# manyeyes/K2TransducerAsr

Hardware: AMD Instinct MI355X
Metric: RTFx (audio-sec/wall-sec) offline Zipformer greedy (higher is better)
Workload: dtype f32

## Files before the change

k2transducerasr_amd/csrc/engine.cpp:

```cpp
#include <cstring>
#include <thread>

#include "engine.h"

#include <climits>
#include <cmath>

namespace k2hip {

namespace {
constexpr int kTailFrames = 19;
}

Engine::Engine(const std::string& weights, const char* overrides, int device) : device_(device) {
    tunables_init_from_env();
    model_.reset(new Model(weights, overrides));
    int n = 0;
    if (hipGetDeviceCount(&n) != hipSuccess || n <= 0)
        failf(K2HIP_ERR_NO_DEVICE, "no HIP device visible: libk2hip has no CPU fallback");
    if (device < 0 || device >= n) failf(K2HIP_ERR_NO_DEVICE, "device %d out of range (have %d)", device, n);
    K2_HIP(hipSetDevice(device));
    model_->upload(device);
    K2_HIP(hipStreamCreateWithFlags(&stream_, hipStreamNonBlocking));
    K2_HIP(hipStreamCreateWithFlags(&stream2_, hipStreamNonBlocking));
// ... 172 lines not shown
    w.dec_table = d_dec_table_;
    return w;
}

void Engine::decoder_table_check(int n_samples, unsigned seed, long long* rows, long long* mismatched) {
    const DecJoinW w = decjoin();
    *rows = 0;
    *mismatched = 0;
    if (!w.dec_table) return;
    const long long V = w.V, n_ctx = (V + 1) * V;
    *rows = n_ctx;
    std::vector<long long> y;
    auto add = [&](long long y0, long long y1) { y.push_back(y0); y.push_back(y1); };
    add(-1, K2HIP_BLANK_ID);
    add(K2HIP_BLANK_ID, K2HIP_BLANK_ID);
    add(-1, V - 1);
    add(V - 1, V - 1);
    unsigned long long st = seed * 6364136223846793005ull + 1442695040888963407ull;
    for (int i = 0; i < n_samples; i++) {
        st = st * 6364136223846793005ull + 1442695040888963407ull;
        const long long cx = (long long)((st >> 20) % (unsigned long long)n_ctx);
        add(cx / V - 1, cx % V);
    }
    const int N = (int)(y.size() / 2);
    long long* d_y = nullptr;
    float* d_out = nullptr;
    K2_HIP(hipMalloc(&d_y, sizeof(long long) * y.size()));
    K2_HIP(hipMalloc(&d_out, sizeof(float) * (size_t)N * w.J));
    std::vector<float> got((size_t)N * w.J), want(w.J);
    try {
        K2_HIP(hipMemcpyAsync(d_y, y.data(), sizeof(long long) * y.size(), hipMemcpyHostToDevice, stream_));
        Ctx t;
        t.stream = stream_;
        decoder_rows_wide(t, w, d_y, N, d_out);
        K2_HIP(hipMemcpyAsync(got.data(), d_out, sizeof(float) * got.size(), hipMemcpyDeviceToHost, stream_));
        K2_HIP(hipStreamSynchronize(stream_));
        for (int n = 0; n < N; n++) {
            const long long row = (y[2 * n] + 1) * V + y[2 * n + 1];
            K2_HIP(copy_blocking(want.data(), w.dec_table + row * w.J, sizeof(float) * w.J, hipMemcpyDeviceToHost));
            for (int k = 0; k < w.J; k++) *mismatched += memcmp(&want[k], &got[(size_t)n * w.J + k], sizeof(float)) != 0;
        }
    } catch (...) {
        (void)hipFree(d_y);
        (void)hipFree(d_out);
        throw;
    }
    (void)hipFree(d_y);
    (void)hipFree(d_out);
}

float* Engine::encoder_embed(const Ctx& c, const float* x, int B, int T, int* T50) {
    const Model& m = *model_;
    const int F0 = 80, T1 = T - 2, T2 = (T1 - 3) / 2 + 1, F2 = (F0 - 3) / 2 + 1, T3 = T2 - 2, F3 = (F2 - 3) / 2 + 1;
    K2_REQUIRE(T3 > 0, "encoder: %d input frames are too few (need >= 9)", T);
    Arena& ar = *c.arena;
    const int D0 = m.cfg().dim[0];
    float* out = ar.take<float>((int64_t)B * T3 * D0);
    int64_t mark = ar.mark();
    float* a1 = ar.take<float>((int64_t)B * T1 * F0 * 8);
    conv0_swoosh(c, x, m.w("encoder_embed.conv.0.weight"), m.w("encoder_embed.conv.0.bias"), a1, B, T, F0);
    c.add_flops(0, 2.0 * B * T1 * (double)F0 * 8 * 9, 0);
    float* a2 = ar.take<float>((int64_t)B * T2 * F2 * 32);
    {
        GemmArgs g;
        g.A = a1; g.W = m.w("encoder_embed.conv.4.weight#ohwi"); g.ldw = 72; g.bias = m.w("encoder_embed.conv.4.bias");
        g.C = a2; g.ldc = 32; g.M = B * T2 * F2; g.N = 32; g.K = 72; g.act = ACT_SWOOSH_R;
        g.cv_Fout = F2; g.cv_Tout = T2; g.cv_Tin = T1; g.cv_Fin = F0; g.cv_C = 8; g.cv_st = 2; g.cv_sf = 2;
        g.seg_len = 24; g.seg_stride = F0 * 8;
        gemm(c, g);
    }
    float* a3 = ar.take<float>((int64_t)B * T3 * F3 * 128);
    {
        GemmArgs g;
        g.A = a2; g.W = m.w("encoder_embed.conv.7.weight#ohwi"); g.ldw = 288; g.bias = m.w("encoder_embed.conv.7.bias");
        g.C = a3; g.ldc = 128; g.M = B * T3 * F3; g.N = 128; g.K = 288; g.act = ACT_SWOOSH_R;
        g.cv_Fout = F3; g.cv_Tout = T3; g.cv_Tin = T2; g.cv_Fin = F2; g.cv_C = 32; g.cv_st = 1; g.cv_sf = 2;
        g.seg_len = 96; g.seg_stride = F2 * 32;
        gemm(c, g);
    }
    const int npix = B * T3 * F3;
    float* dw = ar.take<float>((int64_t)npix * 128);
    dwconv7x7(c, a3, m.w("encoder_embed.convnext.depthwise_conv.weight#kc"), m.w("encoder_embed.convnext.depthwise_conv.bias"),
              dw, B, T3, T3, 3, F3, 128);
    float* hid = ar.take<float>((int64_t)npix * 384);
    linear(c, dw, 128, m.w("encoder_embed.convnext.pointwise_conv1.weight"), m.w("encoder_embed.convnext.pointwise_conv1.bias"),
           hid, 384, npix, 128, 384, ACT_SWOOSH_L);
    linear(c, hid, 384, m.w("encoder_embed.convnext.pointwise_conv2.weight"), m.w("encoder_embed.convnext.pointwise_conv2.bias"),
           a3, 128, npix, 384, 128, ACT_NONE, a3, 128);
    float* lin = ar.take<float>((int64_t)B * T3 * D0);
    linear(c, a3, F3 * 128, m.w("encoder_embed.out.weight#fc"), m.w("encoder_embed.out.bias"), lin, D0, B * T3, F3 * 128, D0);
    biasnorm(c, lin, m.w("encoder_embed.out_norm.bias"), m.w("encoder_embed.out_norm.log_scale"), out, B * T3, D0);
    ar.rewind(mark);
    *T50 = T3;
    return out;
}

const float* Engine::pos_proj_cached(const Ctx& c, int layer, const float* pe, int pe_dim, const float* W, int rows, int ncols) {
    if (c.dry) return nullptr;
    std::lock_guard<std::mutex> lk(cache_mu_);
    const auto key = std::make_pair(layer, rows);
    auto it = pp_cache_.find(key);
    if (it != pp_cache_.end()) return it->second;
    const size_t bytes = sizeof(float) * (size_t)rows * ncols;
    if (pp_cache_bytes_ + bytes > ((size_t)1 << 30)) {
        synchronize();
        for (auto& kv : pp_cache_) (void)hipFree(kv.second);
        pp_cache_.clear();
        pp_cache_bytes_ = 0;
    }
    float* pp = nullptr;
    K2_HIP(hipMalloc(&pp, bytes));
    Ctx plain = c;
    plain.instrument = false;
    plain.gemm_log = nullptr;
    linear(plain, pe, pe_dim, W, nullptr, pp, ncols, rows, pe_dim, ncols);
    K2_HIP(hipStreamSynchronize(c.stream));
    pp_cache_[key] = pp;
    pp_cache_bytes_ += bytes;
    return pp;
}

void Engine::encoder_layer(const Ctx& c, int si, int li, float* x, const float* pe, int B, int T, const LayerTail* tail) {
    const Model& m = *model_;
    const Config& cf = m.cfg();
    const int D = cf.dim[si], F = cf.ff[si], H = cf.heads[si], vh = cf.vhd[si], K = cf.kern[si];
    const int M = B * T, Tp = (T + 3) & ~3, inproj = (2 * cf.qhd[si] + cf.phd[si]) * H, Hc = 3 * D / 4, HV = H * vh;
    char p[96];
    snprintf(p, sizeof p, "encoder.encoders.%d.layers.%d.", si, li);
    auto w = [&](const char* suffix) { return m.w(std::string(p) + suffix); };
    Arena& ar = *c.arena;
    int64_t mark = ar.mark();

    const int F1 = F * 3 / 4, ldcat = F1 + inproj;
    float* cat = ar.take<float>((int64_t)M * ldcat);
    {
        GemmArgs g;
        g.A = x; g.lda = D; g.W = w("#ff1_attn_in.weight"); g.ldw = D; g.bias = w("#ff1_attn_in.bias");
        g.C = cat; g.ldc = ldcat; g.M = M; g.N = ldcat; g.K = D; g.act = ACT_SWOOSH_L; g.act_cols = F1;
        gemm(c, g);
    }
    const float* qkp = cat + F1;
    int gl = li;
    for (int i = 0; i < si; i++) gl += cf.nlayer[i];
    const float* pp = pos_proj_cached(c, gl, pe, cf.pos_dim, w("self_attn_weights.linear_pos.weight"), 2 * T - 1, cf.phd[si] * H);
    float* aw = ar.take<float>((int64_t)H * B * T * Tp);
    attn_scores_softmax(c, qkp, ldcat, pp, aw, B, T, Tp, H);

    float* src = ar.take<float>((int64_t)M * D);
    float* hid = ar.take<float>((int64_t)M * std::max({F * 5 / 4, 3 * Hc, 2 * D}));
    float* tmp = ar.take<float>((int64_t)M * std::max(D, Hc));
    float* tmp2 = ar.take<float>((int64_t)M * std::max(D, Hc));

    auto feed_forward = [&](int k, int Fk, const float* in, float* out) {
        char a[48], b[48], cc[48], d[48];
        snprintf(a, sizeof a, "feed_forward%d.in_proj.weight", k);
        snprintf(b, sizeof b, "feed_forward%d.in_proj.bias", k);
        snprintf(cc, sizeof cc, "feed_forward%d.out_proj.weight", k);
        snprintf(d, sizeof d, "feed_forward%d.out_proj.bias", k);
        linear(c, in, D, w(a), w(b), hid, Fk, M, D, Fk, ACT_SWOOSH_L);
        linear(c, hid, Fk, w(cc), w(d), out, D, M, Fk, D, ACT_NONE, in, D);
    };
    auto self_attn = [&](int k) {
        char a[48], b[48], cc[48], d[48];
        snprintf(a, sizeof a, "self_attn%d.in_proj.weight", k);
        snprintf(b, sizeof b, "self_attn%d.in_proj.bias", k);
        snprintf(cc, sizeof cc, "self_attn%d.out_proj.weight", k);
        snprintf(d, sizeof d, "self_attn%d.out_proj.bias", k);
        linear(c, src, D, w(a), w(b), hid, HV, M, D, HV);
        if (attn_av_out(c, aw, hid, w(cc), w(d), src, B, T, T, Tp, H, vh, D)) return;
        GemmArgs g;
        g.A = aw; g.lda = Tp; g.sA0 = (long long)T * Tp; g.sA1 = (long long)B * T * Tp;
// ... 1276 lines not shown
            g.glu = I(); g.glu_cols = I();
            g.ldm = I(); g.sM0 = L(); g.sM1 = L();
            g.ld_orig = I();
            const int cfg = I(), res_is_C = I();
            const long long oA = L(), oW = L(), oR = L(), oC = L(), oM = L(), oO = L();
            float *A = P(), *W = P(), *bias = P(), *res = P(), *C = P();
            const int* skip = reinterpret_cast<const int*>(P());
            float *mul = P(), *orig = P(), *scale = P();
            int* plan_out = reinterpret_cast<int*>(P());
            K2_REQUIRE(A && W && C && plan_out && buf_bytes[n_bufs - 1] >= 20, "debug_op_run gemm: A, W, C and a plan buffer of 5 ints are needed");
            K2_REQUIRE(!(res_is_C && res), "debug_op_run gemm: res_is_C takes no res buffer");
            K2_REQUIRE(oA >= 0 && oW >= 0 && oR >= 0 && oC >= 0 && oM >= 0 && oO >= 0, "debug_op_run gemm: negative offset");
            if (res_is_C) res = C;
            g.A = A + oA; g.W = W + oW; g.bias = bias; g.res = res ? res + oR : nullptr; g.C = C + oC;
            g.skip_if_zero = skip;
            g.mul = mul ? mul + oM : nullptr;
            g.byp_orig = orig ? orig + oO : nullptr; g.byp_scale = scale;
            GemmForceGuard force(cfg);
            const GemmPlan pl = plan_gemm(g, gemm_force());
            const int rep[5] = {(int)pl.family, pl.idx, pl.BM, pl.BN, pl.mode};
            K2_HIP(copy_blocking(plan_out, rep, sizeof rep, hipMemcpyHostToDevice));
            gemm(c, g);
        } else if (name == "gemm_glu_causal_conv") {
            float *x = P(), *wg = P(), *bg = P(), *pool = P();
            const long long ss = L(), off = L();
            const int* slots = reinterpret_cast<const int*>(P());
            float *wc = P(), *bc = P(), *ww = P(), *bw = P(), *sc = P(), *y = P();
            const int B = I(), Tc = I(), D = I(), K = I();
            int* entry_out = reinterpret_cast<int*>(P());
            K2_REQUIRE(entry_out && buf_bytes[n_bufs - 1] >= 4, "debug_op_run gemm_glu_causal_conv: an entry buffer of 1 int is needed");
            const int entry = glu_conv_ring_entry(B, Tc, D, K);
            K2_HIP(copy_blocking(entry_out, &entry, sizeof entry, hipMemcpyHostToDevice));
            took = gemm_glu_causal_conv(c, x, wg, bg, pool, ss, off, slots, wc, bc, ww, bw, sc, y, B, Tc, D, K);
        } else if (name == "biasnorm") {
            float *x = P(), *bias = P(), *ls = P(), *y = P();
            const int M = I(), D = I();
            biasnorm(c, x, bias, ls, y, M, D);
        } else if (name == "bypass") {
            float *orig = P(), *x = P(), *scale = P(), *y = P();
            const int M = I(), D = I();
            bypass(c, orig, x, scale, y, M, D);
        } else if (name == "biasnorm_bypass") {
            float *x = P(), *orig = P(), *nb = P(), *ls = P(), *scale = P(), *y = P();
            const int M = I(), D = I();
            biasnorm_bypass(c, x, orig, nb, ls, scale, y, M, D);
        } else if (name == "biasnorm_bypass_downsample") {
            float *x = P(), *orig = P(), *nb = P(), *ls = P(), *scale = P(), *y = P(), *bias2 = P(), *xd2 = P();
            const int B = I(), T = I(), D = I(), ds2 = I(), D2 = I();
            biasnorm_bypass_downsample(c, x, orig, nb, ls, scale, y, bias2, xd2, B, T, D, ds2, D2);
        } else if (name == "downsample") {
            float *x = P(), *bias = P(), *y = P();
            const int B = I(), T = I(), D = I(), ds = I(), Din = I();
            downsample(c, x, bias, y, B, T, D, ds, Din);
        } else if (name == "downsample_full") {
            FullDimSegs s;
            s.n = I();
            K2_REQUIRE(s.n >= 1 && s.n <= 8, "debug_op_run downsample_full: %d segments", s.n);
            for (int k = 0; k < s.n; k++) s.ld[k] = I();
            for (int k = 0; k < s.n; k++) s.col1[k] = I();
            s.lz_Td = I(); s.lz_ds = I(); s.lz_Do = I();
            for (int k = 0; k < s.n; k++) s.src[k] = P();
            s.lz_orig = P(); s.lz_xd = P(); s.lz_scale = P();
            float *bias = P(), *y = P();
            const int B = I(), T = I(), D = I(), ds = I();
            downsample_full(c, s, bias, y, B, T, D, ds);
        } else if (name == "upsample_combine") {
            float *orig = P(), *xd = P(), *scale = P(), *y = P();
            const int B = I(), T = I(), Td = I(), D = I(), ds = I(), Dorig = I();
            upsample_combine(c, orig, xd, scale, y, B, T, Td, D, ds, Dorig);
        } else if (name == "upsample_combine_downsample") {
            float *orig = P(), *xd = P(), *scale = P(), *y = P(), *bias2 = P(), *xd2 = P();
            const int B = I(), T = I(), Td = I(), D = I(), ds = I(), Dorig = I(), D2 = I(), ds2 = I();
            upsample_combine_downsample(c, orig, xd, scale, y, bias2, xd2, B, T, Td, D, ds, Dorig, D2, ds2);
        } else if (name == "glu_dwconv1d_swoosh" || name == "glu_dwconv1d_dswish" || name == "dwconv1d_swoosh") {
            float *x = P(), *w = P(), *b = P(), *y = P();
            const int B = I(), T = I(), D = I(), K = I();
            if (name == "glu_dwconv1d_swoosh") glu_dwconv1d_swoosh(c, x, w, b, y, B, T, D, K);
            else if (name == "glu_dwconv1d_dswish") glu_dwconv1d_dswish(c, x, w, b, y, B, T, D, K);
            else dwconv1d_swoosh(c, x, w, b, y, B, T, D, K);
        } else if (name == "dwconv7x7") {
            float *x = P(), *w = P(), *b = P(), *y = P();
            const int B = I(), Tin = I(), Tout = I(), tpad = I(), F = I(), C = I();
            dwconv7x7(c, x, w, b, y, B, Tin, Tout, tpad, F, C);
        } else if (name == "conformer_qprep") {
            float *qkv = P(), *bu = P(), *bv = P(), *qu = P(), *qv = P();
            const int M = I(), D = I();
            const float scaling = F();
            const int ldq = I();
            conformer_qprep(c, qkv, bu, bv, qu, qv, M, D, scaling, ldq);
        } else if (name == "conformer_scores_softmax") {
            float *qu = P(), *qv = P(), *kmat = P();
            const int ldk = I();
            float *pp = P(), *aw = P();
            const int B = I(), H = I(), T = I(), Tp = I(), D = I(), ldq = I();
            float *bu = P(), *bv = P();
            const float scaling = F();
            took = conformer_scores_softmax(c, qu, qv, kmat, ldk, pp, aw, B, H, T, Tp, D, ldq, bu, bv, scaling);
        } else if (name == "conformer_softmax_shift") {
            float *ac = P(), *bd = P();
            const int Z = I(), T = I(), Tp = I(), NPp = I();
            conformer_softmax_shift(c, ac, bd, Z, T, Tp, NPp);
        } else if (name == "conformer_softmax_shift_stream") {
            float *ac = P(), *bd = P();
            const long long* plen = reinterpret_cast<const long long*>(P());
            const int B = I(), H = I(), Tc = I(), left = I(), KLp = I(), NPp = I();
            conformer_softmax_shift_stream(c, ac, bd, plen, B, H, Tc, left, KLp, NPp);
        } else if (name == "slice_rows") {
            float *in = P(), *out = P();
            const int B = I(), Tin = I(), row0 = I(), Tout = I(), D = I();
            slice_rows(c, in, out, B, Tin, row0, Tout, D);
        } else if (name == "dwconv_valid_dswish") {
            float *cat = P(), *w = P(), *bias = P(), *y = P();
            const int B = I(), Tc = I(), D = I(), K = I();
            dwconv_valid_dswish(c, cat, w, bias, y, B, Tc, D, K);
        } else if (name == "z1_pool") {
            float *x = P(), *pool = P();
            const long long ss = L(), avg_off = L(), len_off = L();
            const int* slots = reinterpret_cast<const int*>(P());
            float* out = P();
            const int B = I(), Tc = I(), D = I();
            z1_pool(c, x, pool, ss, avg_off, len_off, slots, out, B, Tc, D);
        } else if (name == "z1_attn") {
            float* qkvp = P();
            const int ld = I();
            float *kcat = P(), *pp = P(), *aw = P();
            const int B = I(), Tc = I(), Lc = I(), KLp = I(), H = I(), A = I();
            z1_attn(c, qkvp, ld, kcat, pp, aw, B, Tc, Lc, KLp, H, A);
        } else if (name == "z1_glu_conv") {
            float *x2 = P(), *pool = P();
            const long long ss = L(), off = L();
            const int* slots = reinterpret_cast<const int*>(P());
            float *w = P(), *bias = P(), *y = P();
            const int B = I(), Tc = I(), D = I(), K = I();
            z1_glu_conv(c, x2, pool, ss, off, slots, w, bias, y, B, Tc, D, K);
        } else if (name == "z1_norm_bypass") {
            float *x = P(), *orig = P(), *le = P(), *bs = P(), *y = P();
            const int M = I(), D = I();
            z1_norm_bypass(c, x, orig, le, bs, y, M, D);
        } else if (name == "z1_attn_downsample") {
            float *x = P(), *query = P(), *y = P();
            const int B = I(), T = I(), Din = I(), ldy = I(), ds = I();
            z1_attn_downsample(c, x, query, y, B, T, Din, ldy, ds);
        } else if (name == "z1_mean") {
            float *x = P(), *mean = P();
            const int B = I(), T = I(), D = I();
            z1_mean(c, x, mean, B, T, D);
        } else if (name == "z1_add_bcast") {
            float *x = P(), *v = P();
            const int B = I(), T = I(), D = I();
            z1_add_bcast(c, x, v, B, T, D);
        } else if (name == "z1_group_rows") {
            float *x = P(), *grp = P();
            const int B = I(), T = I(), Din = I(), ds = I();
            z1_group_rows(c, x, grp, B, T, Din, ds);
        } else if (name == "z1_combine") {
            float* s1 = P();
            const int d1 = I();
            float* s2 = P();
            const int d2 = I();
            float *w1 = P(), *ub = P();
            const int ds = I(), B = I(), T = I(), Td = I();
            float* y = P();
            z1_combine(c, s1, d1, s2, d2, w1, ub, ds, B, T, Td, y);
        } else if (name == "lstm_cell") {
            float* gx = P();
            const long long ldgx = L();
// ... 157 lines not shown
```

k2transducerasr_amd/csrc/gemm.hip:

```cpp
#include <algorithm>
#include <cmath>
#include <cstdlib>
#include <map>
#include <mutex>
#include <type_traits>

#include "kernels.h"

#pragma clang diagnostic ignored "-Winline-asm"

namespace k2hip {

typedef float f32x16 __attribute__((ext_vector_type(16)));
typedef float f32x4 __attribute__((ext_vector_type(4)));

namespace {


__device__ __forceinline__ float fast_softplus(float z) {
    return z > 15.f ? z : __logf(1.0f + __expf(z));
}
__device__ __forceinline__ float apply_act(float v, int act) {
    switch (act) {
        case ACT_SWOOSH_L: return fast_softplus(v - 4.0f) - 0.08f * v - 0.035f;
// ... 1467 lines not shown
    if (ctx.dry) return;
    if (ctx.instrument) K2_HIP(hipEventRecord(ctx.next_event(), ctx.stream));
    const GemmPlan p = plan_gemm(a, gemm_force());
    GemmArgs b = a;
    b.ablate = p.ablate;
    b.xcd_panels = tunables().xcd_panels;
    switch (p.family) {
        case GemmFamily::REG:
            if (p.mode == MODE_CONV) launch_reg<MODE_CONV>(ctx, b, p.idx);
            else if (p.mode == MODE_WKN) launch_reg<MODE_WKN>(ctx, b, p.idx);
            else launch_reg<MODE_PLAIN>(ctx, b, p.idx);
            break;
        case GemmFamily::DMA:
            switch (p.idx) {
#define X(i, bm, bn, wm, wn, nst) case i: launch_dma<bm, bn, wm, wn, nst>(ctx, b); break;
                K2_DMA_TABLE(X)
#undef X
            }
            break;
        case GemmFamily::PIPE:
            switch (p.idx) {
#define X(i, bm, bn, wm, wn, nst) case i: launch_pipe<bm, bn, wm, wn, nst>(ctx, b); break;
                K2_PIPE_TABLE(X)
#undef X
            }
            break;
        case GemmFamily::P16:
            switch (p.idx) {
#define X(i, bm, bn, wm, wn, nst) case i: launch_p16<bm, bn, wm, wn, nst>(ctx, b); break;
                K2_P16_TABLE(X)
#undef X
            }
            break;
        case GemmFamily::RING:
            switch (p.idx) {
#define X(i, bm, bn, ks, nst, lw, pf) case i: launch_ring<bm, bn, ks, nst, lw, pf>(ctx, b); break;
                K2_RING_TABLE(X)
#undef X
            }
            break;
        case GemmFamily::SKINNY3:
            hipLaunchKernelGGL(gemm_f32_mfma_skinny<3>, dim3(cdiv(a.M, 16), 1), dim3(256), 0, ctx.stream, b);
            break;
        case GemmFamily::SKINNY6:
            hipLaunchKernelGGL(gemm_f32_mfma_skinny<6>, dim3(cdiv(a.M, 16), cdiv(a.N, 96)), dim3(256), 0, ctx.stream, b);
            break;
        case GemmFamily::SKINNY6_8:
            hipLaunchKernelGGL((gemm_f32_mfma_skinny<6, 8>), dim3(cdiv(a.M, 16), cdiv(a.N, 96)), dim3(512), 0, ctx.stream, b);
            break;
    }
    K2_HIP(hipGetLastError());
    if (ctx.instrument && ctx.gemm_log)
        ctx.gemm_log->push_back({a.M, a.N, a.K, a.nb0 * a.nb1, a.act, a.res != nullptr, gemm_kind(a, p), 0.f});
    if (ctx.instrument) K2_HIP(hipEventRecord(ctx.next_event(), ctx.stream));
}

bool gemm_glu_causal_conv(const Ctx& ctx, const float* x, const float* wg, const float* bg, float* pool, long long slot_stride, long long off,
                          const int* slots, const float* wc, const float* bc, const float* ww, const float* bw, const float* sc, float* y, int B,
                          int Tc, int D, int K) {
    const int M = B * Tc, N = 2 * D;
    const int entry = glu_conv_ring_entry(B, Tc, D, K);
    if (entry < 0) return false;
    const double fl = 2.0 * M * (double)N * D;
    ctx.add_flops(fl, 2.0 * M * (double)D * (K + (K + 1) / 2), 1);
    if (ctx.dry) return true;
    GemmArgs g;
    g.A = x; g.lda = D; g.W = wg; g.ldw = D; g.bias = bg; g.C = y; g.ldc = D; g.M = M; g.N = N; g.K = D;
    g.cf_pool = pool; g.cf_stride = slot_stride; g.cf_off = off; g.cf_slots = slots;
    g.cf_wc = wc; g.cf_bc = bc; g.cf_ww = ww; g.cf_bw = bw; g.cf_sc = sc; g.cf_Tc = Tc; g.cf_K = K;
    g.xcd_panels = tunables().xcd_panels;
    if (ctx.instrument) K2_HIP(hipEventRecord(ctx.next_event(), ctx.stream));
    if (ctx.instrument && ctx.gemm_log) ctx.gemm_log->push_back({M, N, D, 1, 0, 0, 64, 0.f});
    switch (entry) {
        case 16: launch_ring_conv_entry<16>(ctx, g); break;
        case 17: launch_ring_conv_entry<17>(ctx, g); break;
        case 12: launch_ring_conv_entry<12>(ctx, g); break;
        default: launch_ring_conv_entry<8>(ctx, g); break;
    }
    K2_HIP(hipGetLastError());
    if (ctx.instrument) K2_HIP(hipEventRecord(ctx.next_event(), ctx.stream));
    return true;
}

void linear(const Ctx& ctx, const float* A, int lda, const float* W, const float* bias, float* C, int ldc, int M, int K,
            int N, int act, const float* res, int ldr) {
    GemmArgs g;
    g.A = A; g.lda = lda; g.W = W; g.ldw = K; g.bias = bias; g.C = C; g.ldc = ldc;
    g.M = M; g.N = N; g.K = K; g.act = act; g.res = res; g.ldr = ldr;
    gemm(ctx, g);
}

}
```

k2transducerasr_amd/csrc/kernels.h:

```cpp
#pragma once
#include "common.h"

namespace k2hip {

#ifdef K2HIP_DEV
#define K2HIP_DEV_SWITCH(name, def) int name = def
#else
#define K2HIP_DEV_SWITCH(name, def) static constexpr int name = def
#endif
struct Tunables {
    int no_glu_epilogue = 0;
    int attn_long = 0;
    int no_fused_av = 0;
    int fused_vproj_min_t = 4;
    int no_fused_vproj = 0;
    int no_fused_conv = 0;
    int conformer_gemm_scores = 0;
    int dw7_tiled = 0;
    int dw1d_tt = 0;
    int lstm_seq = 0;
    int greedy_one_part = 0;
    int greedy_parts = 0;
    int beam_launches = 0;
    int beam_parts = 0;
// ... 100 lines not shown

#define K2_PIPE_TABLE(X)                                                                                                       \
    X(0, 128, 64, 64, 32, 3) X(1, 128, 64, 32, 32, 3) X(2, 128, 128, 64, 64, 3) X(3, 128, 128, 64, 32, 3) X(4, 128, 64, 64, 32, 4)  \
    X(5, 64, 64, 32, 32, 3) X(6, 128, 128, 64, 64, 4) X(7, 64, 128, 32, 64, 3) X(8, 128, 128, 32, 32, 3) X(9, 128, 64, 32, 32, 4) \
    X(10, 64, 64, 64, 32, 3) X(11, 64, 64, 32, 64, 3) X(12, 256, 64, 64, 32, 3) X(13, 128, 32, 32, 32, 3) X(14, 128, 32, 64, 32, 3)
#define K2_P16_TABLE(X) X(0, 64, 96, 32, 48, 3) X(1, 128, 96, 64, 48, 3) X(2, 64, 192, 32, 96, 3) X(3, 32, 96, 16, 48, 3)
#define K2_RING_TABLE(X)                                                                                        \
    X(0, 128, 64, 1, 2, 0, 0) X(1, 128, 64, 1, 3, 0, 0) X(2, 128, 64, 1, 2, 0, 1) X(3, 128, 64, 1, 3, 0, 1) X(4, 128, 64, 1, 4, 0, 1)   \
    X(5, 64, 64, 1, 3, 0, 0) X(6, 64, 64, 1, 3, 0, 1) X(7, 64, 64, 1, 4, 0, 1) X(8, 64, 64, 2, 3, 0, 0) X(9, 64, 64, 2, 3, 0, 1)      \
    X(10, 64, 64, 4, 2, 0, 0) X(11, 64, 64, 4, 2, 0, 1) X(12, 32, 64, 2, 3, 0, 0) X(13, 32, 64, 4, 3, 0, 0) X(14, 32, 64, 4, 3, 0, 1)  \
    X(15, 32, 32, 4, 3, 0, 0) X(16, 32, 32, 4, 4, 0, 1) X(17, 64, 32, 4, 3, 0, 0) X(18, 128, 128, 1, 2, 0, 0) X(19, 128, 128, 1, 2, 0, 1) \
    X(20, 64, 128, 1, 3, 0, 0) X(21, 64, 128, 1, 3, 0, 1) X(22, 64, 96, 1, 3, 0, 0) X(23, 64, 96, 1, 3, 0, 1) X(24, 128, 96, 1, 2, 0, 1) \
    X(25, 128, 64, 1, 3, 2, 0) X(26, 128, 64, 1, 3, 2, 1) X(27, 128, 64, 2, 2, 0, 1) X(28, 64, 96, 2, 3, 0, 0) X(29, 64, 96, 2, 2, 0, 0) \
    X(30, 64, 96, 2, 2, 0, 1) X(31, 128, 96, 1, 3, 0, 0) X(32, 128, 96, 1, 3, 0, 1)
struct RingCfg { int BM, BN, KS, NST, LW, PF; };
#define X(i, bm, bn, ks, nst, lw, pf) {bm, bn, ks, nst, lw, pf},
constexpr RingCfg kRing[] = {K2_RING_TABLE(X)};
#undef X
#define K2_DMA_TABLE(X)                                                                                                          \
    X(0, 128, 128, 64, 32, 3) X(5, 128, 64, 32, 32, 2) X(8, 128, 64, 32, 32, 4) X(9, 64, 64, 32, 32, 2) X(10, 64, 64, 32, 32, 3) \
    X(11, 64, 96, 32, 32, 2) X(20, 32, 32, 32, 32, 4) X(21, 32, 64, 32, 32, 4)
#define K2_REG_TABLE(X)                                                                                                           \
    X(0, 128, 128, 64, 32, 32) X(1, 128, 128, 64, 32, 64) X(2, 64, 64, 32, 32, 32) X(3, 64, 64, 32, 32, 64) X(4, 128, 64, 32, 32, 64) \
    X(5, 128, 64, 32, 32, 32) X(12, 128, 32, 32, 32, 32)
enum GemmMode { MODE_PLAIN = 0, MODE_CONV = 1, MODE_WKN = 2 };

enum class GemmFamily { REG, DMA, PIPE, P16, RING, SKINNY3, SKINNY6, SKINNY6_8 };
struct GemmPlan {
    GemmFamily family = GemmFamily::REG;
    int idx = 0;
    int mode = MODE_PLAIN;
    int ablate = 0;
    int BM = 0, BN = 0, waves = 0;
};
struct GemmForce {
    enum Kind { AUTO, CFG, RING, PIPE, P16 } kind = AUTO;
    int idx = -1;
    int ablate = 0;
    bool dma = true;
};
GemmForce decode_gemm_force(int code);
GemmPlan plan_gemm(const GemmArgs& a, const GemmForce& f);
int gemm_kind(const GemmArgs& a, const GemmPlan& p);
int glu_conv_ring_entry(int B, int Tc, int D, int K);
void debug_force_gemm_cfg(int code);
GemmForce gemm_force();
struct GemmForceGuard {
    explicit GemmForceGuard(int code) { debug_force_gemm_cfg(code); }
    ~GemmForceGuard() { debug_force_gemm_cfg(-1); }
    GemmForceGuard(const GemmForceGuard&) = delete;
    GemmForceGuard& operator=(const GemmForceGuard&) = delete;
};
void linear(const Ctx& ctx, const float* A, int lda, const float* W, const float* bias, float* C, int ldc, int M, int K,
            int N, int act = ACT_NONE, const float* res = nullptr, int ldr = 0);

struct RingRef {
    float* pool = nullptr;
    long long slot_stride = 0;
    long long off = 0;
    const int* slots = nullptr;
    const int* chunks = nullptr;
};

void attn_scores_softmax(const Ctx& ctx, const float* qkp, int ld, const float* pp, float* aw, int B, int T, int Tp, int H, int qh = 32,
                         int koff0 = -1, int poff0 = -1);

bool attn_av_out(const Ctx& ctx, const float* aw, const float* v, const float* wout, const float* bias, float* x, int B, int T, int KL, int Tp,
                 int H, int vh, int D);
bool attn_av_out_ring(const Ctx& ctx, const float* aw, const RingRef& vals, const float* newrows, const float* wout, const float* bias, float* x,
                      int B, int T, int KL, int Tp, int H, int vh, int D);
void attn_proj_av_out_ring(const Ctx& ctx, const float* aw, const RingRef& vals, const float* xin, const float* win, const float* bin,
                           const float* wout, const float* bias, float* xout, int B, int T, int KL, int Tp, int H, int vh, int D);

void nonlin_av_out_ring(const Ctx& ctx, const float* aw, const RingRef& cache, const float* hid, int ldh, const float* wout, const float* bias,
                        float* x, int B, int T, int KL, int Tp, int Hc, int D);

void pad_logfloor(const Ctx& ctx, const float* packed, const long long* d_off, const long long* d_len, float* out, int B,
                  long long L);
void pad_logfloor_dense(const Ctx& ctx, const float* feats, long long n_each, float* out, int B, long long L);
void conv0_swoosh(const Ctx& ctx, const float* x, const float* w, const float* b, float* y, int B, int T, int F);
void conv0_pad1_dswish(const Ctx& ctx, const float* x, const float* w, const float* b, float* y, int B, int T, int F);
void dwconv7x7(const Ctx& ctx, const float* x, const float* w_kc, const float* b, float* y, int B, int Tin, int Tout, int tpad,
               int F, int C);
void biasnorm(const Ctx& ctx, const float* x, const float* bias, const float* log_scale, float* y, int M, int D);
void biasnorm_bypass(const Ctx& ctx, const float* x, const float* orig, const float* nbias, const float* log_scale,
                     const float* scale, float* y, int M, int D);
void biasnorm_bypass_downsample(const Ctx& ctx, const float* x, const float* orig, const float* nbias, const float* log_scale, const float* scale,
                                float* y, const float* bias2, float* xd2, int B, int T, int D, int ds2, int D2);
struct LayerTail {
    const float* bias2 = nullptr;
    float* xd2 = nullptr;
    int ds2 = 1, D2 = 0;
};
void bypass(const Ctx& ctx, const float* orig, const float* x, const float* scale, float* y, int M, int D);
void glu_sigmoid(const Ctx& ctx, const float* x, float* y, int M, int D);
void tanh_gate(const Ctx& ctx, const float* x, float* y, int M, int Hc);
void mul_cols(const Ctx& ctx, float* a, const float* x, int ldx, int col0, int M, int N);
void dwconv1d_swoosh(const Ctx& ctx, const float* x, const float* w_kd, const float* b, float* y, int B, int T, int D, int K);
void glu_dwconv1d_swoosh(const Ctx& ctx, const float* x2, const float* w_kd, const float* b, float* y, int B, int T, int D,
                          int K);
void glu_dwconv1d_dswish(const Ctx& ctx, const float* x2, const float* w_kd, const float* b, float* y, int B, int T, int D,
                          int K);
void conv0_nopad_dswish(const Ctx& ctx, const float* x, const float* w, const float* b, float* y, int B, int T, int F);
void lstm_cell(const Ctx& ctx, const float* gx, long long ldgx, const float* gh, int ldgh, float* c, float* hf, int B, int Hh);
void add_inplace(const Ctx& ctx, float* a, const float* b, long long n);
void lstm_cell_rows(const Ctx& ctx, const float* gates, float* c, float* hf, int rows, int Hh);
void lstm_add_frame(const Ctx& ctx, const float* Y, long long SY, const float* hp, long long pstride, int S, float* h, float* x1, int n, int B,
                    int T, int D, int lo, int s);
void lstm_norm_frame(const Ctx& ctx, const float* x1, const float* fp, long long pstride, int S, const float* b2_0, const float* eps0,
                     long long lstride, float* Y, long long SY, int n, int B, int T, int D, int lo, int s);
void gather_rows(const Ctx& ctx, const float* pool, long long slot_stride, long long off, const int* slots, float* out, int B, int width);
void scatter_rows(const Ctx& ctx, float* pool, long long slot_stride, long long off, const int* slots, const float* in, int ldin, int B, int width);
void basicnorm(const Ctx& ctx, const float* x, const float* log_eps, float* y, int M, int D);
void conformer_qprep(const Ctx& ctx, const float* qkv, const float* bias_u, const float* bias_v, float* qu, float* qv, int M,
                     int D, float scaling, int ldq = 0 );
void conformer_softmax_shift_stream(const Ctx& ctx, float* ac, const float* bd, const long long* plen, int B, int H, int Tc, int left,
                                    int KLp, int NPp);
void slice_rows(const Ctx& ctx, const float* in, float* out, int B, int Tin, int row0, int Tout, int D);
void dwconv_valid_dswish(const Ctx& ctx, const float* cat, const float* w_kd, const float* bias, float* y, int B, int Tc, int D, int K);
void conformer_softmax_shift(const Ctx& ctx, float* ac, const float* bd, int Z, int T, int Tp, int NPp);
bool conformer_scores_softmax(const Ctx& ctx, const float* qu, const float* qv, const float* kmat, int ldk, const float* pp, float* aw, int B, int H,
                              int T, int Tp, int D, int ldq = 0, const float* bias_u = nullptr, const float* bias_v = nullptr, float scaling = 1.0f);
void downsample(const Ctx& ctx, const float* x, const float* bias, float* y, int B, int T, int D, int ds, int Din = 0);
void upsample_combine(const Ctx& ctx, const float* orig, const float* xd, const float* scale, float* y, int B, int T,
                      int Td, int D, int ds, int Dorig = 0);
void upsample_combine_downsample(const Ctx& ctx, const float* orig, const float* xd, const float* scale, float* y, const float* bias2,
                                 float* xd2, int B, int T, int Td, int D, int ds, int Dorig, int D2, int ds2);
void convert_channels(const Ctx& ctx, const float* x, float* y, int M, int Din, int Dout);
struct FullDimSegs {
    const float* src[8];
    int ld[8], col1[8], n = 0;
    const float* lz_orig = nullptr;
    const float* lz_xd = nullptr;
    const float* lz_scale = nullptr;
    int lz_Td = 0, lz_ds = 1, lz_Do = 0;
};
void downsample_full(const Ctx& ctx, const FullDimSegs& segs, const float* bias, float* y, int B, int T, int D, int ds);
void copy_cols(const Ctx& ctx, const float* x, int ldx, int xcol0, float* y, int ldy, int ycol0, int M, int n);

struct FbankArgs {
    const float* samples;
    long long n_samples;
    long long utt_stride;
    int n_utts;
    long long n_frames;
    float* feats;
    const float* window;
    const float* melw;
    int frame_len, frame_shift;
    float preemph, input_scale;
    int remove_dc;
    const float* melrange = nullptr;
};
void fbank(const Ctx& ctx, const FbankArgs& a);
void gather_samples(const Ctx& ctx, const float* const* src, const long long* n, float* dst, int B, long long nmax);

struct DecJoinW {
    const float* emb;
    const float* conv;
    int cpg;
    const float* ptab = nullptr;
    const float* dproj_kn;
    const float* dproj_b;
    const float* out_kn;
    const float* out_b;
    const float* dec_table = nullptr;
// ... 205 lines not shown
```

Measured before the change: 23610.

## Fuse ConvNeXt pointwise MLP pair into one persistent MFMA kernel

Replaces the two linear calls of the encoder_embed ConvNeXt block (128->384 with SwooshL, then 384->128 plus residual) with a single persistent kernel. The kernel keeps the 384-wide hidden activations in registers chunk by chunk and streams weight chunks into LDS via double-buffered global_load_lds DMA. It uses fp32 MFMA 32x32x2 and adds the residual in the epilogue. This removes the write and re-read of the npix x 384 hidden buffer and one launch, at the cost of a hand-tuned kernel with inline asm and a fixed channel shape.

Result: no change. 23540 (-0.3%).

```diff
diff --git a/k2transducerasr_amd/csrc/engine.cpp b/k2transducerasr_amd/csrc/engine.cpp
--- a/k2transducerasr_amd/csrc/engine.cpp
+++ b/k2transducerasr_amd/csrc/engine.cpp
@@ -278,11 +278,8 @@
     float* dw = ar.take<float>((int64_t)npix * 128);
     dwconv7x7(c, a3, m.w("encoder_embed.convnext.depthwise_conv.weight#kc"), m.w("encoder_embed.convnext.depthwise_conv.bias"),
               dw, B, T3, T3, 3, F3, 128);
-    float* hid = ar.take<float>((int64_t)npix * 384);
-    linear(c, dw, 128, m.w("encoder_embed.convnext.pointwise_conv1.weight"), m.w("encoder_embed.convnext.pointwise_conv1.bias"),
-           hid, 384, npix, 128, 384, ACT_SWOOSH_L);
-    linear(c, hid, 384, m.w("encoder_embed.convnext.pointwise_conv2.weight"), m.w("encoder_embed.convnext.pointwise_conv2.bias"),
-           a3, 128, npix, 384, 128, ACT_NONE, a3, 128);
+    convnext_pointwise(c, dw, m.w("encoder_embed.convnext.pointwise_conv1.weight"), m.w("encoder_embed.convnext.pointwise_conv1.bias"),
+                       m.w("encoder_embed.convnext.pointwise_conv2.weight"), m.w("encoder_embed.convnext.pointwise_conv2.bias"), a3, npix);
     float* lin = ar.take<float>((int64_t)B * T3 * D0);
     linear(c, a3, F3 * 128, m.w("encoder_embed.out.weight#fc"), m.w("encoder_embed.out.bias"), lin, D0, B * T3, F3 * 128, D0);
     biasnorm(c, lin, m.w("encoder_embed.out_norm.bias"), m.w("encoder_embed.out_norm.log_scale"), out, B * T3, D0);
@@ -1725,6 +1722,15 @@
             float *x = P(), *w = P(), *b = P(), *y = P();
             const int B = I(), Tin = I(), Tout = I(), tpad = I(), F = I(), C = I();
             dwconv7x7(c, x, w, b, y, B, Tin, Tout, tpad, F, C);
+        } else if (name == "convnext_pointwise") {
+            float *x = P(), *W1 = P(), *b1 = P(), *W2 = P(), *b2 = P(), *y = P();
+            const long long M = L();
+            const int max_workgroups = I();
+            const int64_t* nb = buf_bytes + nbuf - 6;
+            K2_REQUIRE(x && W1 && b1 && W2 && b2 && y && M > 0 && nb[0] >= M * 512 && nb[5] >= M * 512 && nb[1] >= 384 * 128 * 4 && nb[2] >= 384 * 4 &&
+                           nb[3] >= 384 * 128 * 4 && nb[4] >= 128 * 4,
+                       "debug_op_run convnext_pointwise: x, y [M, 128], W1 [384, 128], b1 [384], W2 [128, 384], b2 [128] are needed");
+            convnext_pointwise(c, x, W1, b1, W2, b2, y, M, max_workgroups);
         } else if (name == "conformer_qprep") {
             float *qkv = P(), *bu = P(), *bv = P(), *qu = P(), *qv = P();
             const int M = I(), D = I();
diff --git a/k2transducerasr_amd/csrc/gemm.hip b/k2transducerasr_amd/csrc/gemm.hip
--- a/k2transducerasr_amd/csrc/gemm.hip
+++ b/k2transducerasr_amd/csrc/gemm.hip
@@ -1573,6 +1573,156 @@
     return true;
 }
 
+namespace {
+constexpr int CNX_C = 128, CNX_H = 384, CNX_BM = 128, CNX_HC = 32, CNX_NCH = CNX_H / CNX_HC;
+constexpr int CNX_STAGE = 2 * CNX_HC * CNX_C;
+constexpr size_t CNX_LDS = sizeof(float) * (2 * CNX_STAGE + CNX_H + CNX_C);
+
+__global__ __launch_bounds__(256, 2) void k_convnext_pointwise(const float* __restrict__ x, const float* __restrict__ W1,
+                                                               const float* __restrict__ b1, const float* __restrict__ W2,
+                                                               const float* __restrict__ b2, float* y, long long M, int ntiles) {
+    static_assert(CNX_NCH % 2 == 0, "the stage of a chunk is its parity, tile after tile");
+    extern __shared__ __attribute__((aligned(16))) float smem[];
+    float* b1s = smem + 2 * CNX_STAGE;
+    float* b2s = b1s + CNX_H;
+    const int tid = threadIdx.x;
+    const int lane = tid & 63, wave = __builtin_amdgcn_readfirstlane(tid >> 6);
+    const int li = lane & 31, lh = lane >> 5;
+    int tile = blockIdx.x;
+    if (tile >= ntiles) return;
+
+    const unsigned lds_base = (unsigned)(unsigned long long)(__attribute__((address_space(3))) char*)smem;
+    unsigned voff[8], mq[8];
+#pragma unroll
+    for (int q = 0; q < 8; q++) {
+        const int n = wave + 4 * (q & 3);
+        const int cp = lane & 7;
+        if (q < 4) {
+            const int r = 8 * (n & 3) + (lane >> 3);
+            voff[q] = (unsigned)((r * CNX_C + 32 * (n >> 2) + 4 * (cp ^ ((r >> 1) & 7))) * 4);
+        } else {
+            const int r = 8 * n + (lane >> 3);
+            voff[q] = (unsigned)((r * CNX_H + 4 * (cp ^ ((r >> 1) & 7))) * 4);
+        }
+        mq[q] = __builtin_amdgcn_readfirstlane(lds_base + (q < 4 ? 0 : CNX_HC * CNX_C * 4) + n * 1024);
+    }
+#define K2_CNX_DMA(ST_, CH_)                                                                                                   \
+    _Pragma("unroll") for (int q = 0; q < 8; q++) {                                                                            \
+        const unsigned long long src_ = q < 4 ? (unsigned long long)W1 + (unsigned long long)(CH_) * (CNX_HC * CNX_C * 4)      \
+                                              : (unsigned long long)W2 + (unsigned long long)(CH_) * (CNX_HC * 4);             \
+        asm volatile("s_add_u32 m0, %2, %3\n\ts_nop 0\n\tglobal_load_lds_dwordx4 %0, %1"                                        \
+                     :                                                                                                         \
+                     : "v"(voff[q]), "s"(src_), "s"(mq[q]), "n"((ST_) * CNX_STAGE * 4)                                         \
+                     : "memory", "m0", "scc");                                                                                 \
+    }
+#define K2_CNX_LANDED()                     \
+    {                                       \
+        __builtin_amdgcn_s_waitcnt(0x0F70); \
+        asm volatile("" ::: "memory");      \
+    }
+    K2_CNX_DMA(0, 0)
+    for (int i = tid; i < CNX_H + CNX_C; i += 256) b1s[i] = i < CNX_H ? b1[i] : b2[i - CNX_H];
+
+    const float* pf[4];
+#pragma unroll
+    for (int t = 0; t < 4; t++) pf[t] = smem + li * 32 + (((2 * t + lh) ^ ((li >> 1) & 7)) << 2);
+
+    f32x4 xf[16];
+    {
+        const long long row = min((long long)tile * CNX_BM + wave * 32 + li, M - 1);
+        const float* xp = x + row * CNX_C + 4 * lh;
+#pragma unroll
+        for (int g = 0; g < 16; g++) xf[g] = *reinterpret_cast<const f32x4*>(xp + 8 * g);
+    }
+    K2_CNX_LANDED()
+    __syncthreads();
+
+#define K2_CNX_CHUNK(ST_, CH_, NEXT_, LASTX_)                                                                                  \
+    {                                                                                                                          \
+        if (NEXT_) K2_CNX_DMA((ST_) ^ 1, ((CH_) + 1) % CNX_NCH)                                                                \
+        f32x16 h;                                                                                                              \
+        _Pragma("unroll") for (int r = 0; r < 16; r++) h[r] = 0.f;                                                             \
+        _Pragma("unroll") for (int g = 0; g < 16; g++) {                                                                       \
+            const f32x4 a = *reinterpret_cast<const f32x4*>(pf[g & 3] + (ST_) * CNX_STAGE + (g >> 2) * 1024);                  \
+            _Pragma("unroll") for (int e = 0; e < 4; e++) h = __builtin_amdgcn_mfma_f32_32x32x2f32(a[e], xf[g][e], h, 0, 0, 0); \
+        }                                                                                                                      \
+        if (LASTX_) {                                                                                                          \
+            const long long row = min((long long)(tile + (int)gridDim.x) * CNX_BM + wave * 32 + li, M - 1);                    \
+            const float* xp = x + row * CNX_C + 4 * lh;                                                                        \
+            _Pragma("unroll") for (int g = 0; g < 16; g++) xf[g] = *reinterpret_cast<const f32x4*>(xp + 8 * g);                \
+        }                                                                                                                      \
+        _Pragma("unroll") for (int q = 0; q < 4; q++) {                                                                        \
+            const f32x4 bb = *reinterpret_cast<const f32x4*>(b1s + (CH_) * CNX_HC + 8 * q + 4 * lh);                           \
+            _Pragma("unroll") for (int e = 0; e < 4; e++) h[4 * q + e] = apply_act(h[4 * q + e] + bb[e], ACT_SWOOSH_L);        \
+        }                                                                                                                      \
+        _Pragma("unroll") for (int q = 0; q < 4; q++) {                                                                        \
+            f32x4 b[4];                                                                                                        \
+            _Pragma("unroll") for (int j = 0; j < 4; j++)                                                                      \
+                b[j] = *reinterpret_cast<const f32x4*>(pf[q] + (ST_) * CNX_STAGE + CNX_HC * CNX_C + j * 1024);                 \
+            _Pragma("unroll") for (int e = 0; e < 4; e++) _Pragma("unroll") for (int j = 0; j < 4; j++)                        \
+                acc[j] = __builtin_amdgcn_mfma_f32_32x32x2f32(h[4 * q + e], b[j][e], acc[j], 0, 0, 0);                         \
+        }                                                                                                                      \
+                                  \
+        __builtin_amdgcn_sched_barrier(0);                                                                                     \
+        K2_CNX_LANDED()                                                                                                        \
+        __syncthreads();                                                                                                       \
+        __builtin_amdgcn_sched_barrier(0);                                                                                     \
+    }
+
+    for (; tile < ntiles; tile += gridDim.x) {
+        const bool more = tile + (int)gridDim.x < ntiles;
+        f32x16 acc[4];
+#pragma unroll
+        for (int j = 0; j < 4; j++)
+#pragma unroll
+            for (int r = 0; r < 16; r++) acc[j][r] = 0.f;
+        for (int c2 = 0; c2 < CNX_NCH - 2; c2 += 2) {
+            K2_CNX_CHUNK(0, c2, true, false)
+            K2_CNX_CHUNK(1, c2 + 1, true, false)
+        }
+        K2_CNX_CHUNK(0, CNX_NCH - 2, true, false)
+        K2_CNX_CHUNK(1, CNX_NCH - 1, more, more)
+
+        const long long row0 = (long long)tile * CNX_BM + wave * 32 + 4 * lh;
+#pragma unroll
+        for (int j = 0; j < 4; j++) {
+            const int col = 32 * j + li;
+            const float bv = b2s[col];
+            float rv[16];
+#pragma unroll
+            for (int r = 0; r < 16; r++) rv[r] = y[min(row0 + Rows32::off(r), M - 1) * CNX_C + col];
+            float* yp = y + row0 * CNX_C + col;
+            if ((long long)(tile + 1) * CNX_BM <= M) {
+#pragma unroll
+                for (int r = 0; r < 16; r++) yp[Rows32::off(r) * CNX_C] = (acc[j][r] + bv) + rv[r];
+            } else {
+#pragma unroll
+                for (int r = 0; r < 16; r++)
+                    if (row0 + Rows32::off(r) < M) yp[Rows32::off(r) * CNX_C] = (acc[j][r] + bv) + rv[r];
+            }
+        }
+    }
+#undef K2_CNX_CHUNK
+#undef K2_CNX_LANDED
+#undef K2_CNX_DMA
+}
+}
+
+void convnext_pointwise(const Ctx& ctx, const float* x, const float* W1, const float* b1, const float* W2, const float* b2, float* y,
+                        long long M, int max_workgroups) {
+    K2_REQUIRE(M > 0 && max_workgroups >= 0, "convnext_pointwise: %lld rows, at most %d workgroups", M, max_workgroups);
+    ctx.add_flops(0.0, 2.0 * 2.0 * (double)M * CNX_C * CNX_H, 0);
+    if (ctx.dry) return;
+    const long long ntiles = (M + CNX_BM - 1) / CNX_BM;
+    K2_REQUIRE(ntiles < (1ll << 30), "convnext_pointwise: %lld rows are too many", M);
+    long long grid = std::min<long long>(ntiles, 2ll * device_cu_count());
+    if (max_workgroups > 0) grid = std::min<long long>(grid, max_workgroups);
+    static LdsAttrOnce lds_attr;
+    lds_attr.ensure(k_convnext_pointwise, (int)CNX_LDS);
+    hipLaunchKernelGGL(k_convnext_pointwise, dim3((unsigned)grid), dim3(256), CNX_LDS, ctx.stream, x, W1, b1, W2, b2, y, M, (int)ntiles);
+    K2_HIP(hipGetLastError());
+}
+
 void linear(const Ctx& ctx, const float* A, int lda, const float* W, const float* bias, float* C, int ldc, int M, int K,
             int N, int act, const float* res, int ldr) {
     GemmArgs g;
diff --git a/k2transducerasr_amd/csrc/kernels.h b/k2transducerasr_amd/csrc/kernels.h
--- a/k2transducerasr_amd/csrc/kernels.h
+++ b/k2transducerasr_amd/csrc/kernels.h
@@ -206,6 +206,8 @@
 void conv0_pad1_dswish(const Ctx& ctx, const float* x, const float* w, const float* b, float* y, int B, int T, int F);
 void dwconv7x7(const Ctx& ctx, const float* x, const float* w_kc, const float* b, float* y, int B, int Tin, int Tout, int tpad,
                int F, int C);
+void convnext_pointwise(const Ctx& ctx, const float* x, const float* W1, const float* b1, const float* W2, const float* b2, float* y,
+                        long long M, int max_workgroups = 0);
 void biasnorm(const Ctx& ctx, const float* x, const float* bias, const float* log_scale, float* y, int M, int D);
 void biasnorm_bypass(const Ctx& ctx, const float* x, const float* orig, const float* nbias, const float* log_scale,
                      const float* scale, float* y, int M, int D);
```
